# mkocabas/EpipolarPose

Hardware: NVIDIA H100
Metric: multi-view samples/sec (4-view 256x256, bs32) (higher is better)
Workload: dtype f16x3 (fp32 operands split into two fp16 planes, 3-pass error-compensated wgmma f16, f32 accumulate: fp32-grade results)

## Files before the change

epipolarpose_b200/csrc/conv16.cu:

```cuda
#include "split16_common.cuh"

namespace {

constexpr int BM = 128;
constexpr int kThreads16 = 384;
constexpr int kConsumers = 256;
constexpr int kStageBudget = 200 * 1024;
constexpr int kBoxBytes = 16 * 128;

struct Plan16 {
  epb_phase_grid grid;
  int Cout;
  int Wv, Hv;
  int T, CB;
  int n_tiles;
  int accumulate;
  int m_fastest;
  int splits;
  int koff[EPB_MAX_TAPS];
};

struct Maps16 {
  CUtensorMap a[4];
  CUtensorMap w;
  CUtensorMap out;
};

template <int BN>
struct Cfg16 {
  static constexpr int A_PLANE = BM * 128;
  static constexpr int B_PLANE = BN * 128;
  static constexpr int A_BYTES = 2 * A_PLANE;
  static constexpr int B_BYTES = 2 * B_PLANE;
  static constexpr int STAGE = A_BYTES + B_BYTES;
  static constexpr int S_ = kStageBudget / STAGE;
  static constexpr int S = S_ > 6 ? 6 : S_;
  static constexpr int BOX_BYTES = (kConsumers / 32) * kBoxBytes;
  static constexpr int STAT_BYTES = (kConsumers / 32) * 2 * BN * 4;
  static constexpr int SMEM =
      S * STAGE + BOX_BYTES + 1024  + 256  + STAT_BYTES;
  static_assert(SMEM <= 227 * 1024, "shared memory budget");
  static_assert(S >= 2, "ring too shallow");
};

template <int BN, bool SPLIT>
__global__ void __launch_bounds__(kThreads16, 1)
conv16_kernel(const __grid_constant__ Plan16 P, const __grid_constant__ Maps16 maps,
              const float* __restrict__ in_sc, const float* __restrict__ w_sc,
              const float* __restrict__ bias, double* __restrict__ stats) {
  using C = Cfg16<BN>;
  const epb_phase_grid& G = P.grid;
  constexpr int BOXES = C::S * C::STAGE;
  constexpr int CTRL = BOXES + C::BOX_BYTES;
  extern __shared__ uint8_t smem_raw[];
  tc::Ring<C::S, C::STAGE> ring(smem_raw, 0, CTRL, CTRL + 64);
  float* sstat = reinterpret_cast<float*>(ring.sm + CTRL + 256);

  const int warp = threadIdx.x >> 5, lane = threadIdx.x & 31;
  const int KB = P.T * P.CB;
  const int total_tiles = G.tiles * P.n_tiles;
  const int items = SPLIT ? total_tiles * P.splits : total_tiles;
  auto tile_of = [&](int item) { return SPLIT ? item % total_tiles : item; };
  auto kb_lo = [&](int s) { return SPLIT ? (int)((int64_t)s * KB / P.splits) : (s ? KB : 0); };
  auto nt_of = [&](int tile) { return P.m_fastest ? tile / G.tiles : tile % P.n_tiles; };
  auto mt_of = [&](int tile) { return P.m_fastest ? tile % G.tiles : tile / P.n_tiles; };

  if (threadIdx.x == 0) ring.init(1, kConsumers / 32);
  __syncthreads();

  if (warp < 4) {
    if (warp == 0 && lane == 0) {
      for (int v = 0; v < 4; ++v) tc::tma_prefetch_desc(&maps.a[v]);
      tc::tma_prefetch_desc(&maps.w);
      tc::tma_prefetch_desc(&maps.out);
      for (int item = blockIdx.x; item < items; item += gridDim.x) {
        const int tile = tile_of(item), s = SPLIT ? item / total_tiles : 0;
        const int nt = nt_of(tile);
        int w0, h0, n0;
        G.tile_origin(mt_of(tile), w0, h0, n0);
        const int kb0 = kb_lo(s), kb1 = kb_lo(s + 1);
        int t = kb0 / P.CB, cb = kb0 % P.CB;
        for (int kb = kb0; kb < kb1; ++kb) {
          tc::mbar_wait(ring.empty(ring.stage), ring.phase ^ 1);
          const uint32_t fb = ring.full(ring.stage);
          tc::mbar_arrive_expect_tx(fb, C::STAGE);
          const uint32_t a_dst = ring.stage_addr(ring.stage);
          const CUtensorMap* am = &maps.a[G.map[t]];
          const int cx = cb * 64, wx = w0 + G.dwq[t], hx = h0 + G.dhq[t];
          tc::tma_load_5d(a_dst, am, fb, cx, wx, hx, n0, 0);
          tc::tma_load_5d(a_dst + C::A_PLANE, am, fb, cx, wx, hx, n0, 1);
          const uint32_t b_dst = a_dst + C::A_BYTES;
          const int kx = P.koff[t] + cx, rx = nt * BN;
          tc::tma_load_3d(b_dst, &maps.w, fb, kx, rx, 0);
          tc::tma_load_3d(b_dst + C::B_PLANE, &maps.w, fb, kx, rx, 1);
          if (++cb == P.CB) { cb = 0; ++t; }
          ring.advance();
        }
      }
    }
    return;
  }

  const int wgc = (warp >> 2) - 1;
  const int ct = threadIdx.x - 128;
  float* wstat = sstat + (ct >> 5) * 2 * BN;
  const int lc = (lane & 3) * 2;
  const int rb = wgc * 64 + (warp & 3) * 16;
  const int ra = rb + (lane >> 2);
  uint8_t* box = ring.sm + BOXES + (ct >> 5) * kBoxBytes;
  const uint32_t box_addr = tc::smem_u32(box);
  auto chunk = [&](int jj) { return ((2 * jj + ((lane & 3) >> 1)) ^ (lane >> 2)) * 16 + (lane & 1) * 8; };
  const float alpha = in_sc[1] * w_sc[1];
  const int twh = G.tw * G.th;
  if (stats) {
    for (int c = ct; c < (kConsumers / 32) * 2 * BN; c += kConsumers) sstat[c] = 0.f;
    tc::named_sync(1, kConsumers);
  }

  float acc[BN / 2];
  int nt_prev = -1;
  for (int item = blockIdx.x; item < items; item += gridDim.x) {
    const int tile = tile_of(item), s = SPLIT ? item / total_tiles : 0;
    const int nt = nt_of(tile);
    if (stats && nt_prev >= 0 && nt != nt_prev)
      tc::stats_flush<BN, kConsumers / 32>(sstat, ct, nt_prev, P.Cout, stats);
    nt_prev = nt;
#pragma unroll
    for (int i = 0; i < BN / 2; ++i) acc[i] = 0.f;
    for (int kb = kb_lo(s), kb1 = kb_lo(s + 1); kb < kb1; ++kb)
      ring.consume(acc, [&](uint32_t st) {
        const uint32_t a_hi = st + wgc * 64 * 128, b_hi = st + C::A_BYTES;
#pragma unroll
        for (int kk = 0; kk < 4; ++kk)
          tc::mma3_f16<0, 0>(acc, tc::desc_kmajor_sw128(a_hi + kk * 32),
                             tc::desc_kmajor_sw128(a_hi + C::A_PLANE + kk * 32),
                             tc::desc_kmajor_sw128(b_hi + kk * 32),
                             tc::desc_kmajor_sw128(b_hi + C::B_PLANE + kk * 32));
      });
    ring.drain(acc);

    int w0, h0, n0;
    G.tile_origin(mt_of(tile), w0, h0, n0);
    bool srow[2];
#pragma unroll
    for (int h = 0; h < 2; ++h) {
      const int r = ra + 8 * h;
      const int w = w0 + r % G.tw, hh = h0 + (r / G.tw) % G.th, n = n0 + r / twh;
      srow[h] = w < G.Wp && hh < G.Hp && n < G.N;
    }
    const int bx = w0 + rb % G.tw, by = h0 + (rb / G.tw) % G.th, bz = n0 + rb / twh;
    const bool band = SPLIT || (bx < P.Wv && by < P.Hv && bz < G.N);
#pragma unroll
    for (int q = 0; q < BN / 32; ++q) {
      if (lane == 0) tc::tma_store_wait_read<0>();
      __syncwarp();
#pragma unroll
      float v[4][2][2];
#pragma unroll
      for (int jj = 0; jj < 4; ++jj) {
        const int col = nt * BN + 32 * q + 8 * jj + lc;
        float2 b = make_float2(0.f, 0.f);
        if (bias && col < P.Cout) b = *reinterpret_cast<const float2*>(bias + col);
#pragma unroll
        for (int h = 0; h < 2; ++h) {
          v[jj][h][0] = acc[16 * q + 4 * jj + 2 * h] * alpha + b.x;
          v[jj][h][1] = acc[16 * q + 4 * jj + 2 * h + 1] * alpha + b.y;
          *reinterpret_cast<float2*>(box + 128 * ((lane >> 2) + 8 * h) + chunk(jj)) =
              make_float2(v[jj][h][0], v[jj][h][1]);
        }
      }
      tc::fence_proxy_async();
      __syncwarp();
      const int c0 = nt * BN + 32 * q;
      if (lane == 0 && band && c0 < P.Cout) {
        if constexpr (SPLIT) tc::tma_store_4d(&maps.out, box_addr, c0, 0, (mt_of(tile) * BM + rb) / 16, s);
        else if (P.accumulate) tc::tma_reduce_add_4d(&maps.out, box_addr, c0, bx, by, bz);
        else tc::tma_store_4d(&maps.out, box_addr, c0, bx, by, bz);
        tc::tma_store_commit();
      }
      if (stats) {
#pragma unroll
        for (int jj = 0; jj < 4; ++jj) tc::stats_add<BN>(wstat, 32 * q + 8 * jj + lc, v[jj], srow);
      }
    }
  }
  if (stats && nt_prev >= 0) tc::stats_flush<BN, kConsumers / 32>(sstat, ct, nt_prev, P.Cout, stats);
  if (lane == 0) tc::tma_store_wait<0>();
}

struct Reduce16 {
  epb_phase_grid grid;
  int Cout, Wv, Hv, splits;
  int64_t sw, sh, sn;
};

__global__ void __launch_bounds__(256)
conv16_splitk_reduce(const __grid_constant__ Reduce16 R, const float* __restrict__ ws,
                     const float* __restrict__ bias, float* __restrict__ out,
                     double* __restrict__ stats) {
  __shared__ double red[2][8][128];
  const epb_phase_grid& G = R.grid;
  const int tx = threadIdx.x, ty = threadIdx.y;
  const int c = (blockIdx.x * 32 + tx) * 4;
  const bool cok = c < R.Cout;
  const int64_t M = (int64_t)G.N * G.Hp * G.Wp;
  const int64_t split_stride = (int64_t)G.tiles * BM * R.Cout;
  float b[4] = {0.f, 0.f, 0.f, 0.f};
  if (bias && cok)
    for (int e = 0; e < 4; ++e) b[e] = bias[c + e];
  double s1[4] = {0.0, 0.0, 0.0, 0.0}, s2[4] = {0.0, 0.0, 0.0, 0.0};
  if (cok) {
    for (int64_t m = (int64_t)blockIdx.y * 8 + ty; m < M; m += (int64_t)gridDim.y * 8) {
      const int w = (int)(m % G.Wp);
      const int64_t q = m / G.Wp;
      const int h = (int)(q % G.Hp), n = (int)(q / G.Hp);
      const int mt = w / G.tw + G.tiles_w * (h / G.th + G.tiles_h * (n / G.tn));
      const int r = w % G.tw + G.tw * (h % G.th + G.th * (n % G.tn));
      const float* src = ws + ((int64_t)mt * BM + r) * R.Cout + c;
      float4 v = *reinterpret_cast<const float4*>(src);
      for (int s = 1; s < R.splits; ++s) {
        const float4 u = *reinterpret_cast<const float4*>(src + s * split_stride);
        v.x += u.x; v.y += u.y; v.z += u.z; v.w += u.w;
      }
      v.x += b[0]; v.y += b[1]; v.z += b[2]; v.w += b[3];
      if (w < R.Wv && h < R.Hv)
        *reinterpret_cast<float4*>(out + n * R.sn + h * R.sh + w * R.sw + c) = v;
      const float a[4] = {v.x, v.y, v.z, v.w};
      for (int e = 0; e < 4; ++e) {
        s1[e] += a[e];
        s2[e] += (double)a[e] * a[e];
      }
    }
  }
  if (!stats) return;
  for (int e = 0; e < 4; ++e) {
    red[0][ty][tx * 4 + e] = s1[e];
    red[1][ty][tx * 4 + e] = s2[e];
  }
  __syncthreads();
  if (ty == 0 && cok)
    for (int e = 0; e < 4; ++e) {
      double t1 = 0.0, t2 = 0.0;
      for (int y = 0; y < 8; ++y) {
        t1 += red[0][y][tx * 4 + e];
        t2 += red[1][y][tx * 4 + e];
      }
      atomicAdd(stats + c + e, t1);
      atomicAdd(stats + R.Cout + c + e, t2);
    }
}

inline int conv16_bn(int Cout) { return Cout <= 64 ? 64 : 128; }

constexpr int kSplitMinKB = 4;
constexpr int kSplitLongKB = 16;

int conv16_run(const epb_conv_geom* g, const epb_half* in, const float* in_sc, const epb_half* w,
               const float* w_sc, const float* bias, float* out, double* stats, int splits,
               float* ws, epb_stream_t stream) {
  int rc = epb_conv_geom_check(g);
  if (rc) return rc;
  EPB_CHECK_ARG(in && in_sc && w && w_sc && out);
  EPB_CHECK_ARG(g->Cin % 64 == 0 && g->Cout % 4 == 0 && g->Cout >= 4);
  EPB_CHECK_ARG(g->is == 1 || g->is == 2);
  EPB_CHECK_ARG(!(stats && g->accumulate));
  EPB_CHECK_ARG((reinterpret_cast<uintptr_t>(in) & 127) == 0 && (reinterpret_cast<uintptr_t>(w) & 15) == 0);
  EPB_CHECK_ARG((reinterpret_cast<uintptr_t>(out) & 15) == 0 && (reinterpret_cast<uintptr_t>(bias) & 7) == 0);
  Plan16 P;
  Maps16 maps;
  memset(&maps, 0, sizeof(maps));
  bool dense;
  rc = epb_plan_phase_grid(g, in, BM, P.grid, maps.a, dense);
  if (rc) return rc;
  const int64_t Ho = dense ? 1 : g->Ho, Wo = dense ? P.grid.Wp : g->Wo, os = dense ? 1 : g->os;
  const int64_t ph = dense ? 0 : g->ph, pw = dense ? 0 : g->pw;
  P.Cout = g->Cout;
  P.Wv = dense ? P.grid.Wp : (g->Wo - g->pw + g->os - 1) / g->os;
  P.Hv = dense ? 1 : (g->Ho - g->ph + g->os - 1) / g->os;
  P.T = g->T; P.CB = g->Cin / 64; P.accumulate = g->accumulate;
  P.splits = splits;
  float* const view = out + (ph * Wo + pw) * g->Cout;
  if (splits == 1) {
    const int bw = P.grid.tw < 16 ? P.grid.tw : 16;
    const int bh = P.grid.th < 16 / bw ? P.grid.th : 16 / bw;
    const int64_t C4 = (int64_t)g->Cout * 4;
    const cuuint64_t dims[4] = {(cuuint64_t)g->Cout, (cuuint64_t)P.Wv, (cuuint64_t)P.Hv,
                                (cuuint64_t)P.grid.N};
    const cuuint64_t strides[3] = {(cuuint64_t)(os * C4), (cuuint64_t)(os * Wo * C4),
                                   (cuuint64_t)(Ho * Wo * C4)};
    const cuuint32_t box[4] = {32, (cuuint32_t)bw, (cuuint32_t)bh, (cuuint32_t)(16 / (bw * bh))};
    rc = epb_encode_map(&maps.out, CU_TENSOR_MAP_DATA_TYPE_FLOAT32, 4, view, dims, strides, box,
                        CU_TENSOR_MAP_L2_PROMOTION_NONE, "output");
    if (rc) return rc;
  } else {
    const int64_t C4 = (int64_t)g->Cout * 4;
    const cuuint64_t dims[4] = {(cuuint64_t)g->Cout, 16, (cuuint64_t)P.grid.tiles * (BM / 16),
                                (cuuint64_t)splits};
    const cuuint64_t strides[3] = {(cuuint64_t)C4, (cuuint64_t)(16 * C4),
                                   (cuuint64_t)((int64_t)P.grid.tiles * BM * C4)};
    const cuuint32_t box[4] = {32, 16, 1, 1};
    rc = epb_encode_map(&maps.out, CU_TENSOR_MAP_DATA_TYPE_FLOAT32, 4, ws, dims, strides, box,
                        CU_TENSOR_MAP_L2_PROMOTION_NONE, "split-K workspace");
    if (rc) return rc;
  }
  for (int t = 0; t < g->T; ++t) P.koff[t] = g->wt[t] * g->Cin;
  P.m_fastest = stats != nullptr;
  const int bn = conv16_bn(g->Cout);
  P.n_tiles = (g->Cout + bn - 1) / bn;
  const int64_t K = (int64_t)g->Tw * g->Cin;
  const cuuint64_t dims[3] = {(cuuint64_t)K, (cuuint64_t)g->Cout, 2};
  const cuuint64_t strides[2] = {(cuuint64_t)K * 2, (cuuint64_t)K * 2 * g->Cout};
  const cuuint32_t box[3] = {64, (cuuint32_t)bn, 1};
  rc = epb_encode_map(&maps.w, CU_TENSOR_MAP_DATA_TYPE_FLOAT16, 3, w, dims, strides, box,
                      CU_TENSOR_MAP_L2_PROMOTION_L2_256B, "weights");
  if (rc) return rc;
  const int64_t tiles = (int64_t)P.grid.tiles * P.n_tiles;
  cudaStream_t st = as_stream(stream);
  if (splits == 1) {
    const unsigned grid = (unsigned)(tiles < kNumSMs ? tiles : kNumSMs);
    if (bn == 64)
      return tc::launch<conv16_kernel<64, false>>(grid, kThreads16, Cfg16<64>::SMEM, st, P, maps,
                                                  in_sc, w_sc, bias, stats);
    return tc::launch<conv16_kernel<128, false>>(grid, kThreads16, Cfg16<128>::SMEM, st, P, maps,
                                                 in_sc, w_sc, bias, stats);
  }
  P.m_fastest = 0;
  const int64_t items = tiles * splits;
  const unsigned grid = (unsigned)(items < kNumSMs ? items : kNumSMs);
  const float* no_bias = nullptr;
  double* no_stats = nullptr;
  rc = bn == 64 ? tc::launch<conv16_kernel<64, true>>(grid, kThreads16, Cfg16<64>::SMEM, st, P, maps,
                                                      in_sc, w_sc, no_bias, no_stats)
                : tc::launch<conv16_kernel<128, true>>(grid, kThreads16, Cfg16<128>::SMEM, st, P,
                                                       maps, in_sc, w_sc, no_bias, no_stats);
  if (rc) return rc;
  Reduce16 R;
  R.grid = P.grid;
  R.Cout = g->Cout; R.Wv = P.Wv; R.Hv = P.Hv; R.splits = splits;
  R.sw = os * g->Cout; R.sh = os * Wo * g->Cout; R.sn = Ho * Wo * g->Cout;
  const int64_t M = (int64_t)P.grid.N * P.grid.Hp * P.grid.Wp;
  const unsigned gx = (unsigned)((g->Cout + 127) / 128);
  int64_t gy = (M + 7) / 8, cap = 4 * kNumSMs / gx + 1;
  if (gy > cap) gy = cap;
  conv16_splitk_reduce<<<dim3(gx, (unsigned)gy), dim3(32, 8), 0, st>>>(R, ws, bias, view, stats);
  EPB_LAUNCH_CHECK();
  return EPB_OK;
}

}

extern "C" __attribute__((visibility("default"))) int epb_conv16_fprop(
    const epb_conv_geom* g, const epb_half* in, const float* in_sc, const epb_half* w,
    const float* w_sc, const float* bias, float* out, double* stats, epb_stream_t stream) {
  return conv16_run(g, in, in_sc, w, w_sc, bias, out, stats, 1, nullptr, stream);
}

extern "C" __attribute__((visibility("default"))) int epb_conv16_splits(const epb_conv_geom* g,
                                                                          int* splits,
                                                                          long long* ws_floats) {
  int rc = epb_conv_geom_check(g);
  if (rc) return rc;
  EPB_CHECK_ARG(splits && ws_floats && g->Cin % 64 == 0 && g->Cout >= 4);
  epb_phase_grid G;
  bool dense;
  rc = epb_tile_phase_grid(g, BM, G, dense);
  if (rc) return rc;
  const int bn = conv16_bn(g->Cout);
  const int64_t tiles = (int64_t)G.tiles * ((g->Cout + bn - 1) / bn);
  const int64_t kb = (int64_t)g->T * (g->Cin / 64);
  int64_t s = kNumSMs / tiles;
  if (s > kb / kSplitMinKB) s = kb / kSplitMinKB;
  if (s < 4 && kb < kSplitLongKB * s) s = 1;
  if (s < 1) s = 1;
  *splits = (int)s;
  *ws_floats = s > 1 ? s * G.tiles * BM * g->Cout : 0;
  return EPB_OK;
}

extern "C" __attribute__((visibility("default"))) int epb_conv16_fprop_splitk(
    const epb_conv_geom* g, const epb_half* in, const float* in_sc, const epb_half* w,
    const float* w_sc, const float* bias, float* out, double* stats, int splits, float* ws,
    long long ws_floats, epb_stream_t stream) {
  int rc = epb_conv_geom_check(g);
  if (rc) return rc;
  EPB_CHECK_ARG(!g->accumulate);
  EPB_CHECK_ARG(g->Cin % 64 == 0 && splits >= 1 && splits <= g->T * (g->Cin / 64));
  if (splits > 1) {
    epb_phase_grid G;
    bool dense;
    rc = epb_tile_phase_grid(g, BM, G, dense);
    if (rc) return rc;
    EPB_CHECK_ARG(ws && (reinterpret_cast<uintptr_t>(ws) & 15) == 0);
    EPB_CHECK_ARG(ws_floats >= (long long)splits * G.tiles * BM * g->Cout);
  }
  return conv16_run(g, in, in_sc, w, w_sc, bias, out, stats, splits, ws, stream);
}
```

Baseline: 487.0.

## Interleave tile walk across pairs of N-tiles with double-buffered stats accumulators

When tiles are ordered M-fastest, the persistent walk now alternates between two adjacent N-tile columns, so a CTA works on two weight tiles at once. Shared-memory BN statistics are double-buffered, one set per N-tile parity, so stats are flushed only when that set's N-tile changes. The aim is to improve weight reuse and L2 locality and to cut stats flushes. The cost is extra shared memory for stats and a more complex walk, which may shrink pipeline depth for large BN.

Result: no change. 486.8 (median of 6 runs) (-0.0%).

```diff
diff --git a/epipolarpose_b200/csrc/conv16.cu b/epipolarpose_b200/csrc/conv16.cu
--- a/epipolarpose_b200/csrc/conv16.cu
+++ b/epipolarpose_b200/csrc/conv16.cu
@@ -36,7 +36,8 @@
   static constexpr int S_ = kStageBudget / STAGE;
   static constexpr int S = S_ > 6 ? 6 : S_;
   static constexpr int BOX_BYTES = (kConsumers / 32) * kBoxBytes;
-  static constexpr int STAT_BYTES = (kConsumers / 32) * 2 * BN * 4;
+  static constexpr int STAT_SET = (kConsumers / 32) * 2 * BN;
+  static constexpr int STAT_BYTES = 2 * STAT_SET * 4;
   static constexpr int SMEM =
       S * STAGE + BOX_BYTES + 1024  + 256  + STAT_BYTES;
   static_assert(SMEM <= 227 * 1024, "shared memory budget");
@@ -64,6 +65,22 @@
   auto kb_lo = [&](int s) { return SPLIT ? (int)((int64_t)s * KB / P.splits) : (s ? KB : 0); };
   auto nt_of = [&](int tile) { return P.m_fastest ? tile / G.tiles : tile % P.n_tiles; };
   auto mt_of = [&](int tile) { return P.m_fastest ? tile % G.tiles : tile / P.n_tiles; };
+  auto walk = [&](auto&& f) {
+    if (!P.m_fastest) {
+      for (int item = blockIdx.x; item < items; item += gridDim.x) f(item);
+      return;
+    }
+    const int g = gridDim.x, b = blockIdx.x;
+    for (int nt = 0; nt < P.n_tiles; nt += 2) {
+      const int lo = nt * G.tiles, mid = lo + G.tiles;
+      const int hi = nt + 1 < P.n_tiles ? mid + G.tiles : mid;
+      int i0 = lo + (b - lo % g + g) % g, i1 = mid + (b - mid % g + g) % g;
+      while (i0 < mid || i1 < hi) {
+        if (i0 < mid) { f(i0); i0 += g; }
+        if (i1 < hi) { f(i1); i1 += g; }
+      }
+    }
+  };
 
   if (threadIdx.x == 0) ring.init(1, kConsumers / 32);
   __syncthreads();
@@ -73,7 +90,7 @@
       for (int v = 0; v < 4; ++v) tc::tma_prefetch_desc(&maps.a[v]);
       tc::tma_prefetch_desc(&maps.w);
       tc::tma_prefetch_desc(&maps.out);
-      for (int item = blockIdx.x; item < items; item += gridDim.x) {
+      walk([&](int item) {
         const int tile = tile_of(item), s = SPLIT ? item / total_tiles : 0;
         const int nt = nt_of(tile);
         int w0, h0, n0;
@@ -96,14 +113,14 @@
           if (++cb == P.CB) { cb = 0; ++t; }
           ring.advance();
         }
-      }
+      });
     }
     return;
   }
 
   const int wgc = (warp >> 2) - 1;
   const int ct = threadIdx.x - 128;
-  float* wstat = sstat + (ct >> 5) * 2 * BN;
+  float* wstat0 = sstat + (ct >> 5) * 2 * BN;
   const int lc = (lane & 3) * 2;
   const int rb = wgc * 64 + (warp & 3) * 16;
   const int ra = rb + (lane >> 2);
@@ -113,18 +130,20 @@
   const float alpha = in_sc[1] * w_sc[1];
   const int twh = G.tw * G.th;
   if (stats) {
-    for (int c = ct; c < (kConsumers / 32) * 2 * BN; c += kConsumers) sstat[c] = 0.f;
+    for (int c = ct; c < 2 * C::STAT_SET; c += kConsumers) sstat[c] = 0.f;
     tc::named_sync(1, kConsumers);
   }
 
   float acc[BN / 2];
-  int nt_prev = -1;
-  for (int item = blockIdx.x; item < items; item += gridDim.x) {
+  int run_nt[2] = {-1, -1};
+  walk([&](int item) {
     const int tile = tile_of(item), s = SPLIT ? item / total_tiles : 0;
     const int nt = nt_of(tile);
-    if (stats && nt_prev >= 0 && nt != nt_prev)
-      tc::stats_flush<BN, kConsumers / 32>(sstat, ct, nt_prev, P.Cout, stats);
-    nt_prev = nt;
+    const int set = nt & 1;
+    if (stats && run_nt[set] >= 0 && nt != run_nt[set])
+      tc::stats_flush<BN, kConsumers / 32>(sstat + set * C::STAT_SET, ct, run_nt[set], P.Cout, stats);
+    run_nt[set] = nt;
+    float* wstat = wstat0 + set * C::STAT_SET;
 #pragma unroll
     for (int i = 0; i < BN / 2; ++i) acc[i] = 0.f;
     for (int kb = kb_lo(s), kb1 = kb_lo(s + 1); kb < kb1; ++kb)
@@ -183,8 +202,10 @@
         for (int jj = 0; jj < 4; ++jj) tc::stats_add<BN>(wstat, 32 * q + 8 * jj + lc, v[jj], srow);
       }
     }
-  }
-  if (stats && nt_prev >= 0) tc::stats_flush<BN, kConsumers / 32>(sstat, ct, nt_prev, P.Cout, stats);
+  });
+  for (int set = 0; set < 2; ++set)
+    if (stats && run_nt[set] >= 0)
+      tc::stats_flush<BN, kConsumers / 32>(sstat + set * C::STAT_SET, ct, run_nt[set], P.Cout, stats);
   if (lane == 0) tc::tma_store_wait<0>();
 }
 
```
